# BIT-Vision/EventPretrain

Measured on AMD Instinct MI355X. Metric: pretrain samples/sec (masked-ViT step, B=64 224^2), higher is better.
Workload: dtype bf16; 1 GPU; ViT-Base masked modeling (diff-map decoder), 224x224 5-bin voxels, batch=64 per GPU, AdamW step included; global_batch=64, parallelism=dp1

## Files before the change

### eventpretrain_amd/csrc/gemm.hip

```cpp
#include "gemm_common.h"

static int g_gemm_variant = 1;
static int g_gemm_g4_fwd = 0;
static int g_gemm_dbg = 0;
static int g_gemm_wt16 = 1;
static unsigned long long *g_stamp_buf = nullptr;
static long long g_stamp_slots = 0, g_stamp_next = 0;
unsigned long long *evp_gemm_next_stamp_slot() {
  if (!g_stamp_buf || g_stamp_slots <= 0) return nullptr;
  return g_stamp_buf + (size_t)((g_stamp_next++) % g_stamp_slots) * 2 * EVP_STAMP_WGS;
}

namespace {

template <typename T> struct Cfg;
template <> struct Cfg<bf16_t> {
  static constexpr int BK = 64;
  static constexpr int EPC = 8;
  static constexpr int KSTEP = 32;
};
template <> struct Cfg<float> {
  static constexpr int BK = 16;
  static constexpr int EPC = 4;
  static constexpr int KSTEP = 4;
};

template <typename T, bool TR, int ROWS, int BK> struct Img;

template <int ROWS, int BK> struct Img<bf16_t, false, ROWS, BK> {
  static constexpr int BYTES = ROWS * BK * 2;
  static __device__ __forceinline__ int chunk_off(int row, int ch) {
    if (BK == 64) return row * 128 + ((ch ^ (row & 7)) << 4);
    return row * 64 + (ch << 4);
  }
};
template <int ROWS, int BK> struct Img<bf16_t, true, ROWS, BK> {
  static constexpr int BYTES = BK * ROWS * 2;
  static __device__ __forceinline__ int chunk_off(int k, int ch) {
    if (ROWS == 256) return k * 512 + ((ch ^ (((k & 3) << 2) | ((k >> 2) & 3))) << 4);
    if (ROWS == 128) return k * 256 + ((ch ^ (((k & 3) << 2) | ((k >> 2) & 3))) << 4);
    else return k * 128 + ((ch ^ ((((k >> 1) & 1) | (((k >> 3) & 1) << 1)) << 1)) << 4);
  }
};
template <int ROWS, int BK> struct Img<float, false, ROWS, BK> {
  static constexpr int LD = 16 + 1;
  static constexpr int BYTES = ((ROWS * LD * 4 + 15) / 16) * 16;
};
template <int ROWS, int BK> struct Img<float, true, ROWS, BK> {
  static constexpr int LD = ROWS + 16;
  static constexpr int BYTES = 16 * LD * 4;
};

template <typename T, bool TR, int ROWS, int NT, int BK> struct Stage {
  static constexpr int EPC = Cfg<T>::EPC;
  static constexpr int CPR = TR ? ROWS / EPC : BK / EPC;
  static constexpr int NROW = TR ? BK : ROWS;
  static constexpr int NCHUNK = (NROW * CPR + NT - 1) / NT;
  uint4 r[NCHUNK];

  __device__ __forceinline__ void load(__amdgpu_buffer_rsrc_t rs, int ld, int row0, int k0, int nrows, int K, int tid) {
#pragma unroll
    for (int i = 0; i < NCHUNK; ++i) {
      const int cid = tid + i * NT;
      const int lr = cid / CPR, c = cid % CPR;
      const int gr = TR ? row0 + c * EPC : row0 + lr;
      const int gk = TR ? k0 + lr : k0 + c * EPC;
      const bool ok = (NROW * CPR % NT == 0 || cid < NROW * CPR) && gr < nrows && gk < K;
      const int off = ok ? (TR ? gk * ld + gr : gr * ld + gk) * (int)sizeof(T) : (int)0x80000000;
      const u32x4 v = __builtin_amdgcn_raw_buffer_load_b128(rs, off, 0, 0);
      r[i] = make_uint4(v[0], v[1], v[2], v[3]);
    }
  }
  __device__ __forceinline__ void store(char *img, int tid) const {
#pragma unroll
    for (int i = 0; i < NCHUNK; ++i) {
      const int cid = tid + i * NT;
      const int lr = cid / CPR, c = cid % CPR;
      if (NROW * CPR % NT == 0 || cid < NROW * CPR) {
        if constexpr (sizeof(T) == 2) {
          *reinterpret_cast<uint4 *>(img + Img<T, TR, ROWS, BK>::chunk_off(lr, c)) = r[i];
        } else {
          float *p = reinterpret_cast<float *>(img) + lr * Img<T, TR, ROWS, BK>::LD + c * 4;
          if (!TR) {
            p[0] = __uint_as_float(r[i].x); p[1] = __uint_as_float(r[i].y);
            p[2] = __uint_as_float(r[i].z); p[3] = __uint_as_float(r[i].w);
          } else {
            *reinterpret_cast<uint4 *>(p) = r[i];
          }
        }
      }
    }
  }
};
template <bool TR, int ROWS, int NT, int BK> struct GStage {
  static constexpr int PIECES = Img<bf16_t, TR, ROWS, BK>::BYTES / 1024;
  static constexpr int PER_WAVE = PIECES / (NT / 64);
  static_assert(PIECES % (NT / 64) == 0, "tile image must split evenly over the waves");
  __device__ __forceinline__ static void issue(__amdgpu_buffer_rsrc_t rs, int ld, int row0, int k0, int nrows, int K, char *img,
                                               int wave, int lane) {
#pragma unroll
    for (int i = 0; i < PER_WAVE; ++i) {
      const int piece = wave * PER_WAVE + i;
      int gr, gk;
      if (!TR && BK == 64) {
        const int row = piece * 8 + (lane >> 3), pos = lane & 7;
        gr = row0 + row;
        gk = k0 + ((pos ^ (row & 7)) << 3);
      } else if (!TR) {
        gr = row0 + piece * 16 + (lane >> 2);
        gk = k0 + ((lane & 3) << 3);
      } else if (ROWS == 128) {
        const int k = piece * 4 + (lane >> 4), pos = lane & 15;
        gk = k0 + k;
        gr = row0 + ((pos ^ (((k & 3) << 2) | ((k >> 2) & 3))) << 3);
      } else {
        const int k = piece * 8 + (lane >> 3), pos = lane & 7;
        gk = k0 + k;
        gr = row0 + ((pos ^ ((((k >> 1) & 1) | (((k >> 3) & 1) << 1)) << 1)) << 3);
      }
      const bool ok = gr < nrows && gk < K;
      const int off = ok ? (TR ? gk * ld + gr : gr * ld + gk) * 2 : (int)0x80000000;
      __builtin_amdgcn_raw_ptr_buffer_load_lds(rs, (lds_void *)(img + piece * 1024), 16, off, 0, 0, 0);
    }
  }
};

template <bool TR, int ROWS, int BK>
__device__ __forceinline__ bf16x8 frag_bf16(const char *img, int rb, int ks, int lane) {
  const int g = lane >> 4, i = lane & 15;
  if constexpr (!TR) {
    const int row = rb + i;
    const uint4 v = *reinterpret_cast<const uint4 *>(img + Img<bf16_t, false, ROWS, BK>::chunk_off(row, ks * 4 + g));
    return __builtin_bit_cast(bf16x8, v);
  } else {
    const int q = i >> 2, p = i & 3;
    const int k = ks * 32 + 8 * g + q;
    const int ch = (rb >> 3) + (p >> 1);
    const char *a0 = img + Img<bf16_t, true, ROWS, BK>::chunk_off(k, ch) + 8 * (p & 1);
    const char *a1 = img + Img<bf16_t, true, ROWS, BK>::chunk_off(k + 4, ch) + 8 * (p & 1);
    const i16x4 lo = __builtin_amdgcn_ds_read_tr16_b64_v4i16((lds_i16x4 *)(a0));
    const i16x4 hi = __builtin_amdgcn_ds_read_tr16_b64_v4i16((lds_i16x4 *)(a1));
    typedef __attribute__((ext_vector_type(8))) short i16x8;
    i16x8 v;
    v[0] = lo[0]; v[1] = lo[1]; v[2] = lo[2]; v[3] = lo[3];
    v[4] = hi[0]; v[5] = hi[1]; v[6] = hi[2]; v[7] = hi[3];
    return __builtin_bit_cast(bf16x8, v);
  }
}
template <bool TR, int ROWS, int BK>
__device__ __forceinline__ u32x4 frag_bf16_asm(const char *img, int rb, int ks, int lane) {
  const int g = lane >> 4, i = lane & 15;
  if constexpr (!TR) {
    const unsigned a = (unsigned)(uintptr_t)(lds_void *)(img + Img<bf16_t, false, ROWS, BK>::chunk_off(rb + i, ks * 4 + g));
    u32x4 v;
    asm volatile("ds_read_b128 %0, %1" : "=v"(v) : "v"(a) : "memory");
    return v;
  } else {
    const int q = i >> 2, p = i & 3;
    const int k = ks * 32 + 8 * g + q;
    const int ch = (rb >> 3) + (p >> 1);
    const unsigned a0 = (unsigned)(uintptr_t)(lds_void *)(img + Img<bf16_t, true, ROWS, BK>::chunk_off(k, ch) + 8 * (p & 1));
    const unsigned a1 = (unsigned)(uintptr_t)(lds_void *)(img + Img<bf16_t, true, ROWS, BK>::chunk_off(k + 4, ch) + 8 * (p & 1));
    u32x2 lo, hi;
    asm volatile("ds_read_b64_tr_b16 %0, %1" : "=v"(lo) : "v"(a0) : "memory");
    asm volatile("ds_read_b64_tr_b16 %0, %1" : "=v"(hi) : "v"(a1) : "memory");
    return u32x4{lo[0], lo[1], hi[0], hi[1]};
  }
}
__device__ __forceinline__ void tie(u32x4 &x) { asm volatile("" : "+v"(x)); }

template <bool TR, int ROWS>
__device__ __forceinline__ float frag_f32(const char *img, int rb, int ks, int lane) {
  const int g = lane >> 4, i = lane & 15;
  const float *f = reinterpret_cast<const float *>(img);
  if constexpr (!TR) return f[(rb + i) * Img<float, false, ROWS, 16>::LD + ks * 4 + g];
  else return f[(ks * 4 + g) * Img<float, true, ROWS, 16>::LD + rb + i];
}

template <typename TC>
__device__ __noinline__ void epilogue_edge(TC *C, TC *aux, const float *bias, const float *residual, float alpha, int act,
                                           int accumulate, int splitk, int64_t o, int64_t ao, int64_t ro, int n, int nv,
                                           float a0, float a1, float a2, bool fast) {
  for (int e = 0; e < nv; ++e) {
    float x = (e == 0 ? a0 : e == 1 ? a1 : a2) * alpha;
    if (bias) x += bias[n + e];
    if (act == EVP_ACT_GELU || act == EVP_ACT_RELU) {
      if (aux) ElemIO<TC>::st(aux + ao + e, x);
      x = act == EVP_ACT_GELU ? gelu_sel(x, fast) : fmaxf(x, 0.f);
    } else if (act == EVP_ACT_DGELU || act == EVP_ACT_DRELU) {
      const float h = ElemIO<TC>::ld(aux + ao + e);
      x *= act == EVP_ACT_DGELU ? dgelu_sel(h, fast) : (h > 0.f ? 1.f : 0.f);
    }
    if (residual) x += residual[ro + e];
    if (splitk > 1) { atomicAdd(reinterpret_cast<float *>(C) + o + e, x); continue; }
    if (accumulate) x += ElemIO<TC>::ld(C + o + e);
    ElemIO<TC>::st(C + o + e, x);
  }
}

template <typename TC, int EPI>
__device__ __forceinline__ void epi_apply4(float4 a, const GemmParams &p, int64_t coff, int m, int n, float4 bias4, bool fast) {
  TC *C = reinterpret_cast<TC *>(p.C);
  if (n + 3 >= p.N) {
    epilogue_edge<TC>(C, reinterpret_cast<TC *>(p.aux), p.bias, p.residual, p.alpha, p.act, p.accumulate, p.splitk,
                      coff + (int64_t)m * p.ldc + n, coff + (int64_t)m * p.ldaux + n, coff + (int64_t)m * p.ldres + n, n,
                      p.N - n, a.x, a.y, a.z, fast);
    return;
  }
  float4 v = epi_pre4(a, p.alpha, bias4), h = make_float4(0.f, 0.f, 0.f, 0.f);
  const int64_t ao = coff + (int64_t)m * p.ldaux + n;
  if constexpr (EPI == 1) { if (p.aux) st4<TC>(reinterpret_cast<TC *>(p.aux) + ao, v); }
  if constexpr (EPI == 2) h = ld4<TC>(reinterpret_cast<const TC *>(p.aux) + ao);
  v = epi_act4<EPI>(v, h, p.act, fast);
  if (p.residual) v = add4(v, *reinterpret_cast<const float4 *>(p.residual + coff + (int64_t)m * p.ldres + n));
  const int64_t o = coff + (int64_t)m * p.ldc + n;
  if (p.splitk > 1) {
    float *c = reinterpret_cast<float *>(p.C) + o;
    atomicAdd(c + 0, v.x); atomicAdd(c + 1, v.y); atomicAdd(c + 2, v.z); atomicAdd(c + 3, v.w);
    return;
  }
  if (p.accumulate) v = add4(v, ld4<TC>(C + o));
  st4<TC>(C + o, v);
}

template <typename TC, int EPI, typename F> __device__ __forceinline__ bool epi_flags(const GemmParams &p, F f) {
  constexpr bool CAN_ACC = sizeof(TC) == 4 && EPI != 1;
  if (!CAN_ACC && p.accumulate) return false;
  auto on_aux = [&](auto res, auto acc) {
    if constexpr (EPI == 1) {
      if (p.aux) return f(res, acc, std::true_type{});
    }
    f(res, acc, std::false_type{});
  };
  auto on_acc = [&](auto res) {
    if constexpr (CAN_ACC) {
      if (p.accumulate) return on_aux(res, std::true_type{});
    }
    on_aux(res, std::false_type{});
  };
  if (p.residual) on_acc(std::true_type{});
  else on_acc(std::false_type{});
  return true;
}

template <typename TC, int EPI, int NI, bool RES, bool ACC, bool AUXST>
__device__ __forceinline__ void epi_row_fast(const float4 (&a)[NI], const GemmParams &p, const float4 (&bias4)[NI], TC *crow, TC *auxrow,
                                             const float *resrow, bool fast) {
  float4 h[NI] = {}, r[NI], c[NI];
#pragma unroll
  for (int j = 0; j < NI; ++j) {
    if constexpr (EPI == 2) h[j] = ld4<TC>(auxrow + j * 16);
    if constexpr (RES) r[j] = *reinterpret_cast<const float4 *>(resrow + j * 16);
    if constexpr (ACC) c[j] = ld4<TC>(crow + j * 16);
  }
#pragma unroll
  for (int j = 0; j < NI; ++j) {
    float4 v = epi_pre4(a[j], p.alpha, bias4[j]);
    if constexpr (AUXST) st4<TC>(auxrow + j * 16, v);
    v = epi_act4<EPI>(v, h[j], p.act, fast);
    if constexpr (RES) v = add4(v, r[j]);
    if constexpr (ACC) v = add4(v, c[j]);
    st4<TC>(crow + j * 16, v);
  }
}

template <typename TC, int EPI, int MI, int NI, bool RES, bool ACC, bool AUXST>
__device__ __forceinline__ void epilogue_fast(const f32x4 (&acc)[MI][NI], const GemmParams &p, int64_t coff, int mbase, int nbase, bool fast) {
  float4 bias4[NI];
#pragma unroll
  for (int j = 0; j < NI; ++j)
    bias4[j] = p.bias ? *reinterpret_cast<const float4 *>(p.bias + nbase + j * 16) : make_float4(0.f, 0.f, 0.f, 0.f);
  TC *C = reinterpret_cast<TC *>(p.C) + coff + (int64_t)mbase * p.ldc + nbase;
  TC *aux = reinterpret_cast<TC *>(p.aux) + coff + (int64_t)mbase * p.ldaux + nbase;
  const float *res = p.residual + coff + (int64_t)mbase * p.ldres + nbase;
#pragma unroll
  for (int i = 0; i < MI; ++i) {
    float4 a[NI];
#pragma unroll
    for (int j = 0; j < NI; ++j) a[j] = make_float4(acc[i][j][0], acc[i][j][1], acc[i][j][2], acc[i][j][3]);
    if (p.dbg == 2 && i > 0 && a[0].x != 12345.678f) continue;
    epi_row_fast<TC, EPI, NI, RES, ACC, AUXST>(a, p, bias4, C + (int64_t)i * 16 * p.ldc, aux + (int64_t)i * 16 * p.ldaux,
                                                res + (int64_t)i * 16 * p.ldres, fast);
  }
}

template <typename TC, int EPI, int MI, int NI>
__device__ __forceinline__ void epilogue(const f32x4 (&acc)[MI][NI], const GemmParams &p, int64_t coff, int mbase, int nbase, bool fast) {
  if (p.dbg == 1 && acc[0][0][0] != 12345.678f) return;
  const bool interior = mbase + (MI - 1) * 16 < p.M && nbase + (NI - 1) * 16 + 3 < p.N && p.splitk <= 1;
  if (interior && epi_flags<TC, EPI>(p, [&](auto res, auto accu, auto auxst) {
        constexpr bool RES = decltype(res)::value, ACC = decltype(accu)::value, AUXST = decltype(auxst)::value;
        epilogue_fast<TC, EPI, MI, NI, RES, ACC, AUXST>(acc, p, coff, mbase, nbase, fast);
      }))
    return;
  float4 bias4[NI];
#pragma unroll
  for (int j = 0; j < NI; ++j) {
    const int n = nbase + j * 16;
    bias4[j] = (p.bias && n + 3 < p.N) ? *reinterpret_cast<const float4 *>(p.bias + n) : make_float4(0.f, 0.f, 0.f, 0.f);
  }
#pragma unroll
  for (int i = 0; i < MI; ++i) {
    const int m = mbase + i * 16;
    if (m >= p.M) continue;
#pragma unroll
    for (int j = 0; j < NI; ++j) {
      const int n = nbase + j * 16;
      if (n >= p.N) continue;
      epi_apply4<TC, EPI>(make_float4(acc[i][j][0], acc[i][j][1], acc[i][j][2], acc[i][j][3]), p, coff, m, n, bias4[j], fast);
    }
  }
}

template <typename TC, int EPI, int BM, int BN, int NT, bool RES, bool ACC, bool AUXST>
__device__ __forceinline__ void epilogue_lds_rows(const float4 *tile, const GemmParams &p, int64_t coff, int m0, int n, int ch, int r0, float4 bias4,
                                                  bool fast) {
  constexpr int CPR = BN / 4, RPP = NT / CPR, STEPS = BM / RPP;
  static_assert(STEPS % 4 == 0, "rows per thread must come in fours");
  TC *C = reinterpret_cast<TC *>(p.C) + coff + n;
  TC *aux = reinterpret_cast<TC *>(p.aux) + coff + n;
  const float *res = p.residual + coff + n;
#pragma unroll 1
  for (int s = 0; s < STEPS; s += 4) {
    float4 a[4], h[4] = {}, r[4], c[4];
    int m[4];
#pragma unroll
    for (int u = 0; u < 4; ++u) {
      const int row = r0 + (s + u) * RPP;
      m[u] = m0 + row;
      a[u] = tile[row * CPR + (ch ^ (row & 15))];
      if constexpr (EPI == 2) h[u] = ld4<TC>(aux + (int64_t)m[u] * p.ldaux);
      if constexpr (RES) r[u] = *reinterpret_cast<const float4 *>(res + (int64_t)m[u] * p.ldres);
      if constexpr (ACC) c[u] = ld4<TC>(C + (int64_t)m[u] * p.ldc);
    }
#pragma unroll
    for (int u = 0; u < 4; ++u) {
      float4 v = epi_pre4(a[u], p.alpha, bias4);
      if constexpr (AUXST) st4<TC>(aux + (int64_t)m[u] * p.ldaux, v);
      v = epi_act4<EPI>(v, h[u], p.act, fast);
      if constexpr (RES) v = add4(v, r[u]);
      if constexpr (ACC) v = add4(v, c[u]);
      st4<TC>(C + (int64_t)m[u] * p.ldc, v);
    }
  }
}

template <int EPI, int BM, int BN, int NT, bool AUXST>
__device__ __forceinline__ void epilogue_lds_rows8(const float4 *tile, const GemmParams &p, int64_t coff, int m0, int n0, bool fast) {
  constexpr int CPR = BN / 4, CPR8 = BN / 8, RPP = NT / CPR8, STEPS = BM / RPP, G = (STEPS % 4 == 0) ? 4 : 2;
  static_assert(STEPS % G == 0, "rows per thread must come in pairs");
  const int tid = threadIdx.x, ch8 = tid % CPR8, r0 = tid / CPR8, n = n0 + ch8 * 8;
  bf16_t *Cb = reinterpret_cast<bf16_t *>(p.C), *Ab = reinterpret_cast<bf16_t *>(p.aux);
  float4 b0 = make_float4(0.f, 0.f, 0.f, 0.f), b1 = b0;
  if (p.bias) {
    b0 = *reinterpret_cast<const float4 *>(p.bias + n);
    b1 = *reinterpret_cast<const float4 *>(p.bias + n + 4);
  }
#pragma unroll 1
  for (int s = 0; s < STEPS; s += G) {
    float4 a0[G], a1[G];
    uint4 h[G] = {};
    int m[G];
#pragma unroll
    for (int u = 0; u < G; ++u) {
      const int row = r0 + (s + u) * RPP;
      m[u] = m0 + row;
      a0[u] = tile[row * CPR + ((2 * ch8) ^ (row & 15))];
      a1[u] = tile[row * CPR + ((2 * ch8 + 1) ^ (row & 15))];
      if constexpr (EPI == 2) h[u] = *reinterpret_cast<const uint4 *>(Ab + coff + (int64_t)m[u] * p.ldaux + n);
    }
#pragma unroll
    for (int u = 0; u < G; ++u) {
      float4 v0 = epi_pre4(a0[u], p.alpha, b0), v1 = epi_pre4(a1[u], p.alpha, b1);
      if constexpr (AUXST) st8_bf16_wt(Ab, coff + (int64_t)m[u] * p.ldaux + n, v0, v1);
      const float4 h0 = unpack_bf16x4(make_uint2(h[u].x, h[u].y)), h1 = unpack_bf16x4(make_uint2(h[u].z, h[u].w));
      constexpr int SMOOTH = EPI == 2 ? EVP_ACT_DGELU : EVP_ACT_GELU, STEP = EPI == 2 ? EVP_ACT_DRELU : EVP_ACT_RELU;
      if (p.act == SMOOTH) { v0 = epi_act4<EPI>(v0, h0, SMOOTH, fast); v1 = epi_act4<EPI>(v1, h1, SMOOTH, fast); }
      else { v0 = epi_act4<EPI>(v0, h0, STEP, fast); v1 = epi_act4<EPI>(v1, h1, STEP, fast); }
      st8_bf16_wt(Cb, coff + (int64_t)m[u] * p.ldc + n, v0, v1);
    }
  }
}

template <typename TC, int EPI, int BM, int BN, int NT, int MI, int NI>
__device__ __forceinline__ void epilogue_lds(const f32x4 (&acc)[MI][NI], const GemmParams &p, int64_t coff, char *smem, int m0, int n0,
                                             int wrow, int wcol, bool fast) {
  if (p.dbg == 1 && acc[0][0][0] != 12345.678f) return;
  constexpr int CPR = BN / 4;
  static_assert(CPR >= 16 && NT % CPR == 0, "tile too narrow for the chunk swizzle");
  const int tid = threadIdx.x, lane = tid & 63, li = lane & 15, lg = lane >> 4;
  float4 *tile = reinterpret_cast<float4 *>(smem);
#pragma unroll
  for (int i = 0; i < MI; ++i)
#pragma unroll
    for (int j = 0; j < NI; ++j) {
      const int row = wrow + i * 16 + li, ch = (wcol >> 2) + j * 4 + lg;
      tile[row * CPR + (ch ^ (row & 15))] = make_float4(acc[i][j][0], acc[i][j][1], acc[i][j][2], acc[i][j][3]);
    }
  __syncthreads();
  if constexpr (sizeof(TC) == 2 && BN % 8 == 0 && (BM % (NT / (BN / 8))) == 0 && (BM / (NT / (BN / 8))) % 2 == 0) {
    if (p.c_wt16 && m0 + BM <= p.M && n0 + BN <= p.N && !p.residual && !p.accumulate && p.splitk <= 1 && (EPI != 2 || p.aux)) {
      if (EPI == 1 && p.aux) epilogue_lds_rows8<EPI, BM, BN, NT, true>(tile, p, coff, m0, n0, fast);
      else epilogue_lds_rows8<EPI, BM, BN, NT, false>(tile, p, coff, m0, n0, fast);
      return;
    }
  }
  const int ch = tid % CPR, r0 = tid / CPR;
  const int n = n0 + ch * 4;
  if (n >= p.N) return;
  const float4 bias4 = (p.bias && n + 3 < p.N) ? *reinterpret_cast<const float4 *>(p.bias + n) : make_float4(0.f, 0.f, 0.f, 0.f);
  constexpr int RPP = NT / CPR;
  const bool interior = m0 + BM <= p.M && n + 3 < p.N && p.splitk <= 1;
  if (interior && epi_flags<TC, EPI>(p, [&](auto res, auto accu, auto auxst) {
        constexpr bool RES = decltype(res)::value, ACC = decltype(accu)::value, AUXST = decltype(auxst)::value;
        epilogue_lds_rows<TC, EPI, BM, BN, NT, RES, ACC, AUXST>(tile, p, coff, m0, n, ch, r0, bias4, fast);
      }))
    return;
  for (int r = r0; r < BM; r += RPP) {
    const int m = m0 + r;
    if (m >= p.M) break;
    epi_apply4<TC, EPI>(tile[r * CPR + (ch ^ (r & 15))], p, coff, m, n, bias4, fast);
  }
}

template <typename T, typename TC, int EPI, bool TA, bool TB, int BM, int BN, int WM, int WN, bool GLDS, int STAGES, int BK>
__device__ __forceinline__ void gemm_body(const GemmParams &p, const int tile_m, const int tile_n, const int bz, const int kslice) {
  constexpr int NT = WM * WN * 64;
  constexpr int KSTEP = Cfg<T>::KSTEP;
  constexpr int WTM = BM / WM, WTN = BN / WN, MI = WTM / 16, NI = WTN / 16;
  constexpr int A_BYTES = Img<T, TA, BM, BK>::BYTES, B_BYTES = Img<T, TB, BN, BK>::BYTES;
  extern __shared__ __attribute__((aligned(16))) char smem[];

  const int tid = threadIdx.x, lane = tid & 63, wave = tid >> 6;
  const int wm = wave / WN, wn = wave % WN;
  const int m0 = tile_m * BM, n0 = tile_n * BN;
  const int b0 = bz / p.batch1, b1 = bz % p.batch1;
  const T *A = reinterpret_cast<const T *>(p.A) + b0 * p.sA0 + b1 * p.sA1;
  const T *B = reinterpret_cast<const T *>(p.B) + b0 * p.sB0 + b1 * p.sB1;
  const __amdgpu_buffer_rsrc_t rsA = __builtin_amdgcn_make_buffer_rsrc(const_cast<T *>(A), 0, 0x7FFFFFFF, 0x00020000);
  const __amdgpu_buffer_rsrc_t rsB = __builtin_amdgcn_make_buffer_rsrc(const_cast<T *>(B), 0, 0x7FFFFFFF, 0x00020000);
  const int lda = (int)p.lda, ldb = (int)p.ldb;

  f32x4 acc[MI][NI];
#pragma unroll
  for (int i = 0; i < MI; ++i)
#pragma unroll
    for (int j = 0; j < NI; ++j) acc[i][j] = f32x4{0.f, 0.f, 0.f, 0.f};

  const int kbeg = kslice * p.k_per_split;
  const int kend = (kbeg + p.k_per_split < p.K) ? kbeg + p.k_per_split : p.K;
  const int ntiles = (kend - kbeg + BK - 1) / BK;

  auto compute_tile = [&](const char *ia, const char *ib) {
#pragma unroll
    for (int ks = 0; ks < BK / KSTEP; ++ks) {
      if constexpr (sizeof(T) == 2) {
        bf16x8 af[MI], bf[NI];
#pragma unroll
        for (int i = 0; i < MI; ++i) af[i] = frag_bf16<TA, BM, BK>(ia, wm * WTM + i * 16, ks, lane);
#pragma unroll
        for (int j = 0; j < NI; ++j) bf[j] = frag_bf16<TB, BN, BK>(ib, wn * WTN + j * 16, ks, lane);
#pragma unroll
        for (int i = 0; i < MI; ++i)
#pragma unroll
          for (int j = 0; j < NI; ++j)
            acc[i][j] = __builtin_amdgcn_mfma_f32_16x16x32_bf16(bf[j], af[i], acc[i][j], 0, 0, 0);
      } else {
        float af[MI], bf[NI];
#pragma unroll
        for (int i = 0; i < MI; ++i) af[i] = frag_f32<TA, BM>(ia, wm * WTM + i * 16, ks, lane);
#pragma unroll
        for (int j = 0; j < NI; ++j) bf[j] = frag_f32<TB, BN>(ib, wn * WTN + j * 16, ks, lane);
#pragma unroll
        for (int i = 0; i < MI; ++i)
#pragma unroll
          for (int j = 0; j < NI; ++j)
            acc[i][j] = __builtin_amdgcn_mfma_f32_16x16x4f32(bf[j], af[i], acc[i][j], 0, 0, 0);
      }
    }
  };

  auto compute_tile_asm = [&](const char *ia, const char *ib) {
    if constexpr (sizeof(T) == 2) {
      constexpr int KS = BK / KSTEP;
      static_assert(KS == 1 || KS == 2, "lgkmcnt literals below");
      u32x4 af[KS][MI], bf[KS][NI];
#pragma unroll
      for (int ks = 0; ks < KS; ++ks) {
#pragma unroll
        for (int i = 0; i < MI; ++i) af[ks][i] = frag_bf16_asm<TA, BM, BK>(ia, wm * WTM + i * 16, ks, lane);
#pragma unroll
        for (int j = 0; j < NI; ++j) bf[ks][j] = frag_bf16_asm<TB, BN, BK>(ib, wn * WTN + j * 16, ks, lane);
      }
#pragma unroll
      for (int ks = 0; ks < KS; ++ks) {
        constexpr int PER_KS = (TA ? 2 : 1) * MI + (TB ? 2 : 1) * NI;
        if (ks + 1 < KS && PER_KS <= 15) {
          if constexpr (PER_KS == 8) asm volatile("s_waitcnt lgkmcnt(8)" ::: "memory");
          else if constexpr (PER_KS == 12) asm volatile("s_waitcnt lgkmcnt(12)" ::: "memory");
          else asm volatile("s_waitcnt lgkmcnt(0)" ::: "memory");
        } else {
          asm volatile("s_waitcnt lgkmcnt(0)" ::: "memory");
        }
#pragma unroll
        for (int i = 0; i < MI; ++i) tie(af[ks][i]);
#pragma unroll
        for (int j = 0; j < NI; ++j) tie(bf[ks][j]);
#pragma unroll
        for (int i = 0; i < MI; ++i)
#pragma unroll
          for (int j = 0; j < NI; ++j)
            acc[i][j] = __builtin_amdgcn_mfma_f32_16x16x32_bf16(__builtin_bit_cast(bf16x8, bf[ks][j]), __builtin_bit_cast(bf16x8, af[ks][i]),
                                                                acc[i][j], 0, 0, 0);
      }
    }
  };

  if constexpr (GLDS) {
    using GA = GStage<TA, BM, NT, BK>;
    using GB = GStage<TB, BN, NT, BK>;
    constexpr int INFLIGHT = GA::PER_WAVE + GB::PER_WAVE;
    static_assert(INFLIGHT == 8 || INFLIGHT == 7 || INFLIGHT == 6 || INFLIGHT == 4, "add the vmcnt literal for this tile shape");
    auto wait_all_but_newest_tile = [] {
      if constexpr (INFLIGHT == 8) asm volatile("s_waitcnt vmcnt(8)" ::: "memory");
      else if constexpr (INFLIGHT == 7) asm volatile("s_waitcnt vmcnt(7)" ::: "memory");
      else if constexpr (INFLIGHT == 6) asm volatile("s_waitcnt vmcnt(6)" ::: "memory");
      else asm volatile("s_waitcnt vmcnt(4)" ::: "memory");
    };
    constexpr int STAGE_BYTES = A_BYTES + B_BYTES;
    if constexpr (STAGES == 2) {
      GA::issue(rsA, lda, m0, kbeg, p.M, kend, smem, wave, lane);
      GB::issue(rsB, ldb, n0, kbeg, p.N, kend, smem + A_BYTES, wave, lane);
      for (int t = 0; t < ntiles; ++t) {
        char *cur = smem + (t & 1) * STAGE_BYTES;
        char *nxt = smem + ((t + 1) & 1) * STAGE_BYTES;
        if (t + 1 < ntiles) {
          GA::issue(rsA, lda, m0, kbeg + (t + 1) * BK, p.M, kend, nxt, wave, lane);
          GB::issue(rsB, ldb, n0, kbeg + (t + 1) * BK, p.N, kend, nxt + A_BYTES, wave, lane);
          wait_all_but_newest_tile();
        } else {
          asm volatile("s_waitcnt vmcnt(0)" ::: "memory");
        }
        __builtin_amdgcn_s_barrier();
        compute_tile_asm(cur, cur + A_BYTES);
        asm volatile("s_waitcnt lgkmcnt(0)" ::: "memory");
        __builtin_amdgcn_s_barrier();
      }
    } else {
      GA::issue(rsA, lda, m0, kbeg, p.M, kend, smem, wave, lane);
      GB::issue(rsB, ldb, n0, kbeg, p.N, kend, smem + A_BYTES, wave, lane);
      if (ntiles > 1) {
        GA::issue(rsA, lda, m0, kbeg + BK, p.M, kend, smem + STAGE_BYTES, wave, lane);
        GB::issue(rsB, ldb, n0, kbeg + BK, p.N, kend, smem + STAGE_BYTES + A_BYTES, wave, lane);
      }
      int st = 0;
      for (int t = 0; t < ntiles; ++t) {
        if (t + 1 < ntiles) wait_all_but_newest_tile();
        else asm volatile("s_waitcnt vmcnt(0)" ::: "memory");
        __builtin_amdgcn_s_barrier();
        if (t + 2 < ntiles) {
          const int s2 = st == 0 ? 2 : st - 1;
          GA::issue(rsA, lda, m0, kbeg + (t + 2) * BK, p.M, kend, smem + s2 * STAGE_BYTES, wave, lane);
          GB::issue(rsB, ldb, n0, kbeg + (t + 2) * BK, p.N, kend, smem + s2 * STAGE_BYTES + A_BYTES, wave, lane);
        }
        const char *cur = smem + st * STAGE_BYTES;
        compute_tile_asm(cur, cur + A_BYTES);
        asm volatile("s_waitcnt lgkmcnt(0)" ::: "memory");
        st = st == 2 ? 0 : st + 1;
      }
      __builtin_amdgcn_s_barrier();
    }
  } else {
    Stage<T, TA, BM, NT, BK> sa;
    Stage<T, TB, BN, NT, BK> sb;
    sa.load(rsA, lda, m0, kbeg, p.M, kend, tid);
    sb.load(rsB, ldb, n0, kbeg, p.N, kend, tid);
    sa.store(smem, tid);
    sb.store(smem + A_BYTES, tid);
    __syncthreads();
    for (int t = 0; t < ntiles; ++t) {
      char *cur = smem + (t & 1) * (A_BYTES + B_BYTES);
      char *nxt = smem + ((t + 1) & 1) * (A_BYTES + B_BYTES);
      const bool more = (t + 1) < ntiles;
      if (more) {
        sa.load(rsA, lda, m0, kbeg + (t + 1) * BK, p.M, kend, tid);
        sb.load(rsB, ldb, n0, kbeg + (t + 1) * BK, p.N, kend, tid);
      }
      compute_tile(cur, cur + A_BYTES);
      if (more) {
        sa.store(nxt, tid);
        sb.store(nxt + A_BYTES, tid);
      }
      __syncthreads();
    }
  }

  if (p.dbg == 3 && p.stamp && tid == 0 && gridDim.x * gridDim.y * gridDim.z <= (unsigned)EVP_STAMP_WGS)
    p.stamp[2 * (blockIdx.x + gridDim.x * (blockIdx.y + gridDim.y * blockIdx.z))] =
        ~(unsigned long long)__builtin_amdgcn_s_memrealtime();
  const int64_t coff = b0 * p.sC0 + b1 * p.sC1;
  const int li = lane & 15, lg = lane >> 4;
  if constexpr (STAGES * (A_BYTES + B_BYTES) >= BM * BN * 4 && EPI == 0 && sizeof(TC) == 4) {
    if (p.splitk > 1) {
      float *tile = reinterpret_cast<float *>(smem);
#pragma unroll
      for (int i = 0; i < MI; ++i)
#pragma unroll
        for (int j = 0; j < NI; ++j) {
          const int r = wm * WTM + i * 16 + li, c = wn * WTN + j * 16 + lg * 4;
          *reinterpret_cast<float4 *>(tile + r * BN + c) =
              make_float4(acc[i][j][0] * p.alpha, acc[i][j][1] * p.alpha, acc[i][j][2] * p.alpha, acc[i][j][3] * p.alpha);
        }
      __syncthreads();
      float *C = reinterpret_cast<float *>(p.C) + coff;
      for (int e = tid; e < BM * BN; e += NT) {
        const int r = e / BN, c = e % BN;
        if (m0 + r < p.M && n0 + c < p.N) atomicAdd(C + (int64_t)(m0 + r) * p.ldc + n0 + c, tile[e]);
      }
      return;
    }
  }
  const bool fast = sizeof(T) == 2;
  if constexpr (sizeof(T) == 2 && STAGES * (A_BYTES + B_BYTES) >= BM * BN * 4 && BN >= 64) {
    epilogue_lds<TC, EPI, BM, BN, NT, MI, NI>(acc, p, coff, smem, m0, n0, wm * WTM, wn * WTN, fast);
  } else {
    epilogue<TC, EPI, MI, NI>(acc, p, coff, m0 + wm * WTM + li, n0 + wn * WTN + lg * 4, fast);
  }
}

template <typename T, typename TC, int EPI, bool TA, bool TB, int BM, int BN, int WM, int WN, bool GLDS, int STAGES, int BK, int MINW>
__global__ __launch_bounds__(WM *WN * 64, MINW) void gemm_kernel(const GemmParams p) {
  int tile_m, tile_n;
  const unsigned wg = blockIdx.x + gridDim.x * (blockIdx.y + gridDim.y * blockIdx.z);
  stamp_begin(p.stamp, wg, gridDim.x * gridDim.y * gridDim.z);
  map_tile(gridDim.x, blockIdx.x, p.tiles_m, tile_m, tile_n);
  gemm_body<T, TC, EPI, TA, TB, BM, BN, WM, WN, GLDS, STAGES, BK>(p, tile_m, tile_n, blockIdx.z, blockIdx.y);
  stamp_end(p.stamp, wg, gridDim.x * gridDim.y * gridDim.z);
}

template <int BM, int BN>
__global__ __launch_bounds__(256) void gemm_grouped_tn_kernel(const GroupedProblem *__restrict__ probs, const GroupedItem *__restrict__ items,
                                                              unsigned long long *stamp) {
  const GroupedItem it = items[blockIdx.x];
  if (it.prob < 0) return;
  stamp_begin(stamp, blockIdx.x, gridDim.x);
  const GroupedProblem g = probs[it.prob];
  GemmParams p;
  p.M = g.M; p.N = g.N; p.K = g.K;
  p.A = g.A; p.lda = g.lda; p.sA0 = 0; p.sA1 = 0;
  p.B = g.B; p.ldb = g.ldb; p.sB0 = 0; p.sB1 = 0;
  p.C = g.C; p.c_dtype = EVP_F32; p.ldc = g.ldc; p.sC0 = 0; p.sC1 = 0;
  p.batch1 = 1; p.alpha = 1.0f; p.bias = nullptr; p.act = EVP_ACT_NONE; p.aux = nullptr; p.ldaux = 0;
  p.residual = nullptr; p.ldres = 0; p.accumulate = g.accumulate; p.tiles_m = 0; p.splitk = 1; p.dbg = 0; p.colsum = nullptr; p.colsum_acc = 0; p.stamp = nullptr; p.c_wt16 = 0;
  p.k_per_split = (g.K + 63) / 64 * 64;
  gemm_body<bf16_t, float, 0, true, true, BM, BN, 2, 2, true, 2, 64>(p, it.tile_m, it.tile_n, 0, 0);
  stamp_end(stamp, blockIdx.x, gridDim.x);
}

template <typename T, typename TC, int EPI, bool TA, bool TB, int BM, int BN, int WM, int WN, bool GLDS, int STAGES, int BK = Cfg<T>::BK,
          int MINW = 1>
int launch(const evp_gemm_desc *d, hipStream_t s) {
  GemmParams p;
  p.M = d->M; p.N = d->N; p.K = d->K;
  p.A = d->A; p.lda = d->lda; p.sA0 = d->strideA0; p.sA1 = d->strideA1;
  p.B = d->B; p.ldb = d->ldb; p.sB0 = d->strideB0; p.sB1 = d->strideB1;
  p.C = d->C; p.c_dtype = d->c_dtype; p.ldc = d->ldc; p.sC0 = d->strideC0; p.sC1 = d->strideC1;
  p.batch1 = d->batch1 > 0 ? d->batch1 : 1;
  p.alpha = d->alpha; p.bias = d->bias; p.act = d->act; p.aux = d->aux; p.ldaux = d->ldaux;
  p.residual = d->residual; p.ldres = d->ldres; p.accumulate = d->accumulate; p.dbg = g_gemm_dbg; p.colsum = nullptr; p.colsum_acc = 0; p.stamp = evp_gemm_next_stamp_slot();
  p.tiles_m = (d->M + BM - 1) / BM;
  const int tiles_n = (d->N + BN - 1) / BN;
  const int nb = (d->batch0 > 0 ? d->batch0 : 1) * p.batch1;
  {
    const int64_t span = (int64_t)d->M * (d->ldc > d->ldaux ? d->ldc : d->ldaux) * 2;
    p.c_wt16 = (g_gemm_wt16 && d->c_dtype == EVP_BF16 && nb == 1 && span < 0x7FFFFFFFLL && d->ldc % 8 == 0 && (!d->aux || d->ldaux % 8 == 0) &&
                ((uintptr_t)d->C & 15) == 0 && ((uintptr_t)d->aux & 15) == 0 && (!d->bias || ((uintptr_t)d->bias & 15) == 0)) ? 1 : 0;
  }
  constexpr int BKc = BK;
  int splitk = d->splitk;
  const bool can_split = d->c_dtype == EVP_F32 && !d->bias && d->act == EVP_ACT_NONE && !d->residual && !d->aux && nb == 1;
  if (splitk == 0) {
    splitk = 1;
    const int tiles = p.tiles_m * tiles_n;
    const int ktiles = (d->K + BKc - 1) / BKc;
    if (can_split && d->transA && tiles < 384 && ktiles >= 16) {
      splitk = (512 + tiles - 1) / tiles;
      if (splitk > ktiles / 8) splitk = ktiles / 8;
      if (splitk < 1) splitk = 1;
    }
  }
  if (!can_split) splitk = 1;
  {
    const int ktiles = (d->K + BKc - 1) / BKc;
    const int per = (ktiles + splitk - 1) / splitk;
    p.k_per_split = per * BKc;
    splitk = (ktiles + per - 1) / per;
    p.splitk = splitk;
  }
  if (splitk > 1 && !d->accumulate) {
    hipError_t e = evp_zero2d_async(d->C, (size_t)d->ldc * 4, (size_t)d->N * 4, (size_t)d->M, s);
    if (e != hipSuccess) { evp_set_error("evp_gemm: memset for split-K failed: %s", hipGetErrorString(e)); return EVP_ELAUNCH; }
  }
  constexpr int smem = STAGES * (Img<T, TA, BM, BK>::BYTES + Img<T, TB, BN, BK>::BYTES);
  auto k = gemm_kernel<T, TC, EPI, TA, TB, BM, BN, WM, WN, GLDS, STAGES, BK, MINW>;
  static bool attr_done = false;
  if (!attr_done) {
    if (smem > 48 * 1024) {
      hipError_t e = hipFuncSetAttribute(reinterpret_cast<const void *>(k), hipFuncAttributeMaxDynamicSharedMemorySize, smem);
      if (e != hipSuccess) {
        evp_set_error("evp_gemm: hipFuncSetAttribute(%d) failed: %s", smem, hipGetErrorString(e));
        return EVP_ELAUNCH;
      }
    }
    attr_done = true;
  }
  dim3 grid((unsigned)(p.tiles_m * tiles_n), (unsigned)splitk, (unsigned)nb);
  hipLaunchKernelGGL(k, grid, dim3(WM * WN * 64), smem, s, p);
  EVP_CHECK_LAUNCH("evp_gemm");
  return EVP_OK;
}


template <typename T, typename TC, int EPI, bool TA, bool TB> int pick_tile(const evp_gemm_desc *d, hipStream_t s) {
  int tile = d->tile;
  const int64_t nb = (int64_t)(d->batch0 > 0 ? d->batch0 : 1) * (d->batch1 > 0 ? d->batch1 : 1);
  if (tile == 0) {
    if constexpr (sizeof(T) == 2 && !TA) {
      if (g_gemm_g4_fwd && g_gemm_variant != 2) {
        const int shape = evp_g4_gemm_pick(d);
        if ((shape == 20 && (g_gemm_g4_fwd & 1)) || (shape == 22 && (g_gemm_g4_fwd & 2))) return evp_g4_gemm(d, s, shape, g_gemm_dbg);
      }
    }
    const int64_t t128 = (int64_t)((d->M + 127) / 128) * ((d->N + 127) / 128) * nb;
    const bool splittable = d->transA && d->c_dtype == EVP_F32 && !d->bias && d->act == EVP_ACT_NONE && !d->residual &&
                            !d->aux && nb == 1 && d->K >= 2048;
    tile = (d->M >= 128 && d->N >= 128 && (t128 >= 192 || splittable)) ? 1 : 2;
    if constexpr (sizeof(T) == 2 && !TA) {
      const int64_t t96 = (int64_t)((d->M + 95) / 96) * ((d->N + 127) / 128) * nb;
      if (tile == 1 && g_gemm_variant != 2 && nb == 1 && t128 > 256 && t96 <= 512) tile = 4;
    }
  }
  if (tile == 6 || tile == 7 || tile == 8 || tile == 12 || tile == 30 || tile == 31) {
    evp_set_error("evp_gemm: tile %d (256x256 ring / persistent / stream-K variants of rounds 1-4) was removed; see DESIGN.md section 4", tile);
    return EVP_EUNSUPPORTED;
  }
  if constexpr (sizeof(T) == 2) {
    if (tile == 9) {
      if constexpr (TA && TB && EPI == 0 && std::is_same<TC, float>::value) {
        if (nb != 1 || d->K % 32 != 0 || d->K < 96 || d->bias || d->residual || d->aux || d->alpha != 1.0f || d->splitk > 1 ||
            d->lda % 8 != 0 || d->ldb % 8 != 0) {
          evp_set_error("evp_gemm: tile 9 (G4) needs transA, transB, f32 C, K %% 32 == 0, K >= 96, no batch / epilogue extras");
          return EVP_ESHAPE;
        }
        return evp_g4_gemm_tn(d, s);
      } else {
        evp_set_error("evp_gemm: tile 9 (G4) is built for the weight-gradient layout (transA = transB = 1, f32 C) only");
        return EVP_EUNSUPPORTED;
      }
    }
    if (tile >= 20 && tile <= 22) {
      if constexpr (!TA) return evp_g4_gemm(d, s, tile, g_gemm_dbg);
      evp_set_error("evp_gemm: tiles 20-22 need A row-major");
      return EVP_EUNSUPPORTED;
    }
  }
  if constexpr (sizeof(T) == 2) {
    if (g_gemm_variant != 2) {
      if (tile == 4) return launch<T, TC, EPI, TA, TB, 96, 128, 2, 2, true, 2>(d, s);
      if (tile == 1) return launch<T, TC, EPI, TA, TB, 128, 128, 2, 2, true, 2>(d, s);
      return launch<T, TC, EPI, TA, TB, 64, 64, 2, 2, true, 2>(d, s);
    }
  }
  if (tile == 1 || tile >= 3) return launch<T, TC, EPI, TA, TB, 128, 128, 2, 2, false, 2>(d, s);
  return launch<T, TC, EPI, TA, TB, 64, 64, 2, 2, false, 2>(d, s);
}

template <typename T, typename TC> int pick_layout(const evp_gemm_desc *d, hipStream_t s) {
  const int epi = (d->act == EVP_ACT_GELU || d->act == EVP_ACT_RELU) ? 1 : (d->act == EVP_ACT_DGELU || d->act == EVP_ACT_DRELU) ? 2 : 0;
  if (epi == 0) {
    if (!d->transA && !d->transB) return pick_tile<T, TC, 0, false, false>(d, s);
    if (!d->transA && d->transB) return pick_tile<T, TC, 0, false, true>(d, s);
    if (d->transA && d->transB) return pick_tile<T, TC, 0, true, true>(d, s);
    evp_set_error("evp_gemm: layout transA=1,transB=0 is not used on this path and not built");
    return EVP_EUNSUPPORTED;
  }
  if (epi == 1 && !d->transA && !d->transB) return pick_tile<T, TC, 1, false, false>(d, s);
  if (epi == 2 && !d->transA && d->transB) return pick_tile<T, TC, 2, false, true>(d, s);
  evp_set_error("evp_gemm: activation epilogue %d is only built for its own layout (forward: NT, backward: transB)", d->act);
  return EVP_EUNSUPPORTED;
}

template <typename T> int pick_ctype(const evp_gemm_desc *d, hipStream_t s) {
  if (d->c_dtype == EVP_F32) return pick_layout<T, float>(d, s);
  if constexpr (sizeof(T) == 2) return pick_layout<T, bf16_t>(d, s);
  evp_set_error("evp_gemm: bf16 output needs bf16 operands");
  return EVP_EUNSUPPORTED;
}

}

extern "C" int evp_gemm_grouped_tn_bf16(const void *problems, const void *items, int n_items, void *stream) {
  EVP_CHECK_ARG(problems && items && n_items > 0, EVP_EINVAL, "evp_gemm_grouped_tn_bf16: bad argument");
  auto k = gemm_grouped_tn_kernel<128, 128>;
  constexpr int smem = 2 * (Img<bf16_t, true, 128, 64>::BYTES + Img<bf16_t, true, 128, 64>::BYTES);
  static bool attr_done = false;
  if (!attr_done) {
    hipError_t e = hipFuncSetAttribute(reinterpret_cast<const void *>(k), hipFuncAttributeMaxDynamicSharedMemorySize, smem);
    EVP_CHECK_ARG(e == hipSuccess, EVP_ELAUNCH, "evp_gemm_grouped_tn_bf16: hipFuncSetAttribute failed: %s", hipGetErrorString(e));
    attr_done = true;
  }
  hipLaunchKernelGGL(k, dim3((unsigned)n_items), dim3(256), smem, (hipStream_t)stream,
                     reinterpret_cast<const GroupedProblem *>(problems), reinterpret_cast<const GroupedItem *>(items), evp_gemm_next_stamp_slot());
  EVP_CHECK_LAUNCH("evp_gemm_grouped_tn_bf16");
  return EVP_OK;
}

extern "C" int evp_gemm_set_stamp_buffer(void *buf, long long n_slots) {
  g_stamp_buf = reinterpret_cast<unsigned long long *>(buf);
  g_stamp_slots = buf ? n_slots : 0;
  g_stamp_next = 0;
  return EVP_OK;
}
extern "C" long long evp_gemm_stamp_count(void) { return g_stamp_next; }

extern "C" int evp_gemm_set_variant(int v) {
  const int old = g_gemm_variant;
  if (v >= 100 && v <= 103) g_gemm_dbg = v - 100;
  if (v == 18 || v == 19) g_gemm_wt16 = v - 18;
  if (v == 1 || v == 2) g_gemm_variant = v;
  if (v >= 10 && v <= 13) g_gemm_g4_fwd = v == 11 ? 3 : v == 10 ? 0 : v - 11;
  return old;
}

extern "C" int evp_gemm(const evp_gemm_desc *d, void *stream) {
  EVP_CHECK_ARG(d != nullptr, EVP_EINVAL, "evp_gemm: null descriptor");
  EVP_CHECK_ARG(d->A && d->B && d->C, EVP_EINVAL, "evp_gemm: null operand");
  EVP_CHECK_ARG(d->M > 0 && d->N > 0 && d->K > 0, EVP_ESHAPE, "evp_gemm: M,N,K must be positive (%d,%d,%d)", d->M, d->N, d->K);
  EVP_CHECK_ARG(d->dtype == EVP_F32 || d->dtype == EVP_BF16, EVP_EINVAL, "evp_gemm: bad dtype %d", d->dtype);
  EVP_CHECK_ARG(d->c_dtype == EVP_F32 || d->c_dtype == EVP_BF16, EVP_EINVAL, "evp_gemm: bad c_dtype %d", d->c_dtype);
  const int epc = d->dtype == EVP_BF16 ? 8 : 4;
  EVP_CHECK_ARG(d->lda % epc == 0 && d->ldb % epc == 0, EVP_ESHAPE,
                "evp_gemm: lda/ldb must be multiples of %d elements (got %lld, %lld)", epc, (long long)d->lda, (long long)d->ldb);
  EVP_CHECK_ARG(((uintptr_t)d->A & 15) == 0 && ((uintptr_t)d->B & 15) == 0, EVP_EINVAL, "evp_gemm: A/B must be 16-byte aligned");
  EVP_CHECK_ARG(d->strideA0 % epc == 0 && d->strideA1 % epc == 0 && d->strideB0 % epc == 0 && d->strideB1 % epc == 0,
                EVP_ESHAPE, "evp_gemm: batch strides of A/B must be multiples of %d elements", epc);
  EVP_CHECK_ARG(!d->accumulate || d->c_dtype == EVP_F32, EVP_EINVAL, "evp_gemm: accumulate needs an f32 C");
  {
    const int64_t es = d->dtype == EVP_BF16 ? 2 : 4;
    const int64_t spanA = (int64_t)(d->transA ? d->K : d->M) * d->lda * es, spanB = (int64_t)(d->transB ? d->K : d->N) * d->ldb * es;
    EVP_CHECK_ARG(spanA < 0x7FFFFFFFLL && spanB < 0x7FFFFFFFLL, EVP_ESHAPE,
                  "evp_gemm: one batch's operand must span < 2 GiB (32-bit buffer offsets)");
  }
  EVP_CHECK_ARG((d->act != EVP_ACT_DGELU && d->act != EVP_ACT_DRELU) || d->aux, EVP_EINVAL, "evp_gemm: dgelu/drelu need aux");
  hipStream_t s = reinterpret_cast<hipStream_t>(stream);
  return d->dtype == EVP_BF16 ? pick_ctype<bf16_t>(d, s) : pick_ctype<float>(d, s);
}
```

Baseline: 5955 samples/s.

## Add 512-thread paired GEMM tiles for large bf16 problems

Adds 256x128, 128x256 and 192x128 bf16 GEMM tiles run by 8 waves, with a 3-stage LDS-DMA ring when B is row-major. By default (pair=1) only the 96x128 case is promoted to the 192x128 tile, for large non-transposed-B GEMMs with K>=1536 such as the MLP fc2. The point is more operand reuse per workgroup and fewer redundant global loads. In exchange the workgroups use more LDS and registers, so fewer fit per CU, and LDS sizing now accounts for the epilogue staging tile.

```diff
diff --git a/eventpretrain_amd/csrc/gemm.hip b/eventpretrain_amd/csrc/gemm.hip
--- a/eventpretrain_amd/csrc/gemm.hip
+++ b/eventpretrain_amd/csrc/gemm.hip
@@ -2,6 +2,7 @@
 
 static int g_gemm_variant = 1;
 static int g_gemm_g4_fwd = 0;
+static int g_gemm_pair = 1;
 static int g_gemm_dbg = 0;
 static int g_gemm_wt16 = 1;
 static unsigned long long *g_stamp_buf = nullptr;
@@ -36,6 +37,7 @@
 };
 template <int ROWS, int BK> struct Img<bf16_t, true, ROWS, BK> {
   static constexpr int BYTES = BK * ROWS * 2;
+  static_assert(ROWS != 192, "no chunk XOR defined for a 192-wide transposed image: the 192x128 tile takes A row-major only");
   static __device__ __forceinline__ int chunk_off(int k, int ch) {
     if (ROWS == 256) return k * 512 + ((ch ^ (((k & 3) << 2) | ((k >> 2) & 3))) << 4);
     if (ROWS == 128) return k * 256 + ((ch ^ (((k & 3) << 2) | ((k >> 2) & 3))) << 4);
@@ -109,6 +111,10 @@
       } else if (!TR) {
         gr = row0 + piece * 16 + (lane >> 2);
         gk = k0 + ((lane & 3) << 3);
+      } else if (ROWS == 256) {
+        const int k = piece * 2 + (lane >> 5), pos = lane & 31;
+        gk = k0 + k;
+        gr = row0 + ((pos ^ (((k & 3) << 2) | ((k >> 2) & 3))) << 3);
       } else if (ROWS == 128) {
         const int k = piece * 4 + (lane >> 4), pos = lane & 15;
         gk = k0 + k;
@@ -423,12 +429,15 @@
   }
 }
 
+constexpr int lds_bytes(int ring, int parked, int nt) { return nt == 512 && parked > ring ? parked : ring; }
+
 template <typename T, typename TC, int EPI, bool TA, bool TB, int BM, int BN, int WM, int WN, bool GLDS, int STAGES, int BK>
 __device__ __forceinline__ void gemm_body(const GemmParams &p, const int tile_m, const int tile_n, const int bz, const int kslice) {
   constexpr int NT = WM * WN * 64;
   constexpr int KSTEP = Cfg<T>::KSTEP;
   constexpr int WTM = BM / WM, WTN = BN / WN, MI = WTM / 16, NI = WTN / 16;
   constexpr int A_BYTES = Img<T, TA, BM, BK>::BYTES, B_BYTES = Img<T, TB, BN, BK>::BYTES;
+  constexpr int LDS_BYTES = lds_bytes(STAGES * (A_BYTES + B_BYTES), BM * BN * 4, NT);
   extern __shared__ __attribute__((aligned(16))) char smem[];
 
   const int tid = threadIdx.x, lane = tid & 63, wave = tid >> 6;
@@ -520,11 +529,12 @@
     using GA = GStage<TA, BM, NT, BK>;
     using GB = GStage<TB, BN, NT, BK>;
     constexpr int INFLIGHT = GA::PER_WAVE + GB::PER_WAVE;
-    static_assert(INFLIGHT == 8 || INFLIGHT == 7 || INFLIGHT == 6 || INFLIGHT == 4, "add the vmcnt literal for this tile shape");
+    static_assert(INFLIGHT == 8 || INFLIGHT == 7 || INFLIGHT == 6 || INFLIGHT == 5 || INFLIGHT == 4, "add the vmcnt literal for this tile shape");
     auto wait_all_but_newest_tile = [] {
       if constexpr (INFLIGHT == 8) asm volatile("s_waitcnt vmcnt(8)" ::: "memory");
       else if constexpr (INFLIGHT == 7) asm volatile("s_waitcnt vmcnt(7)" ::: "memory");
       else if constexpr (INFLIGHT == 6) asm volatile("s_waitcnt vmcnt(6)" ::: "memory");
+      else if constexpr (INFLIGHT == 5) asm volatile("s_waitcnt vmcnt(5)" ::: "memory");
       else asm volatile("s_waitcnt vmcnt(4)" ::: "memory");
     };
     constexpr int STAGE_BYTES = A_BYTES + B_BYTES;
@@ -600,7 +610,7 @@
         ~(unsigned long long)__builtin_amdgcn_s_memrealtime();
   const int64_t coff = b0 * p.sC0 + b1 * p.sC1;
   const int li = lane & 15, lg = lane >> 4;
-  if constexpr (STAGES * (A_BYTES + B_BYTES) >= BM * BN * 4 && EPI == 0 && sizeof(TC) == 4) {
+  if constexpr (LDS_BYTES >= BM * BN * 4 && EPI == 0 && sizeof(TC) == 4) {
     if (p.splitk > 1) {
       float *tile = reinterpret_cast<float *>(smem);
 #pragma unroll
@@ -621,7 +631,7 @@
     }
   }
   const bool fast = sizeof(T) == 2;
-  if constexpr (sizeof(T) == 2 && STAGES * (A_BYTES + B_BYTES) >= BM * BN * 4 && BN >= 64) {
+  if constexpr (sizeof(T) == 2 && LDS_BYTES >= BM * BN * 4 && BN >= 64) {
     epilogue_lds<TC, EPI, BM, BN, NT, MI, NI>(acc, p, coff, smem, m0, n0, wm * WTM, wn * WTN, fast);
   } else {
     epilogue<TC, EPI, MI, NI>(acc, p, coff, m0 + wm * WTM + li, n0 + wn * WTN + lg * 4, fast);
@@ -701,7 +711,7 @@
     hipError_t e = evp_zero2d_async(d->C, (size_t)d->ldc * 4, (size_t)d->N * 4, (size_t)d->M, s);
     if (e != hipSuccess) { evp_set_error("evp_gemm: memset for split-K failed: %s", hipGetErrorString(e)); return EVP_ELAUNCH; }
   }
-  constexpr int smem = STAGES * (Img<T, TA, BM, BK>::BYTES + Img<T, TB, BN, BK>::BYTES);
+  constexpr int smem = lds_bytes(STAGES * (Img<T, TA, BM, BK>::BYTES + Img<T, TB, BN, BK>::BYTES), BM * BN * 4, WM * WN * 64);
   auto k = gemm_kernel<T, TC, EPI, TA, TB, BM, BN, WM, WN, GLDS, STAGES, BK, MINW>;
   static bool attr_done = false;
   if (!attr_done) {
@@ -738,6 +748,10 @@
     if constexpr (sizeof(T) == 2 && !TA) {
       const int64_t t96 = (int64_t)((d->M + 95) / 96) * ((d->N + 127) / 128) * nb;
       if (tile == 1 && g_gemm_variant != 2 && nb == 1 && t128 > 256 && t96 <= 512) tile = 4;
+      if (g_gemm_pair && g_gemm_variant != 2 && nb == 1 && t128 > 256) {
+        if (tile == 4 && (g_gemm_pair > 1 || (!TB && d->K >= 1536))) tile = 42;
+        else if (tile == 1 && g_gemm_pair > 1) tile = g_gemm_pair == 2 ? 40 : 41;
+      }
     }
   }
   if (tile == 6 || tile == 7 || tile == 8 || tile == 12 || tile == 30 || tile == 31) {
@@ -764,6 +778,18 @@
       return EVP_EUNSUPPORTED;
     }
   }
+  if (tile >= 40 && tile <= 42) {
+    if constexpr (sizeof(T) == 2 && !TA) {
+      if (g_gemm_variant != 2) {
+        constexpr int PST = TB ? 2 : 3;
+        if (tile == 40) return launch<T, TC, EPI, TA, TB, 256, 128, 4, 2, true, PST>(d, s);
+        if (tile == 41) return launch<T, TC, EPI, TA, TB, 128, 256, 2, 4, true, PST>(d, s);
+        return launch<T, TC, EPI, TA, TB, 192, 128, 4, 2, true, PST>(d, s);
+      }
+    }
+    evp_set_error("evp_gemm: tiles 40-42 (paired 256x128 / 128x256 / 192x128) need bf16 operands, A row-major and LDS-DMA staging");
+    return EVP_EUNSUPPORTED;
+  }
   if constexpr (sizeof(T) == 2) {
     if (g_gemm_variant != 2) {
       if (tile == 4) return launch<T, TC, EPI, TA, TB, 96, 128, 2, 2, true, 2>(d, s);
@@ -827,6 +853,7 @@
   const int old = g_gemm_variant;
   if (v >= 100 && v <= 103) g_gemm_dbg = v - 100;
   if (v == 18 || v == 19) g_gemm_wt16 = v - 18;
+  if (v >= 40 && v <= 43) g_gemm_pair = v - 40;
   if (v == 1 || v == 2) g_gemm_variant = v;
   if (v >= 10 && v <= 13) g_gemm_g4_fwd = v == 11 ? 3 : v == 10 ? 0 : v - 11;
   return old;
```

After: 5952 samples/s (median of 3 runs). Within noise of the previous version (-0.1%).
